# ReadAlongs/SoundSwallower

Hardware: AMD Instinct MI355X
Metric: senone-frames/sec (en-us PTM) (higher is better)
Workload: dtype f32+i32

## Files before the change

### include/ssw_amd.h

```cpp
#ifndef SSW_AMD_H
#define SSW_AMD_H

#include <stddef.h>
#include <stdint.h>

#ifdef __cplusplus
extern "C" {
#endif

#define SSW_ABI_VERSION 2

typedef struct ssw_config_s {
    double logbase;
    double varfloor;
    double mixwfloor;
    double tmatfloor;
    int32_t topn;
    int32_t ds;
    int32_t aw;
    int32_t device;
} ssw_config_t;
#define SSW_DEVICE_NONE (-2)

void ssw_config_defaults(ssw_config_t *cfg);
// ... 3 lines not shown
typedef struct ssw_model_s ssw_model_t;

ssw_model_t *ssw_model_load(const char *mdef, const char *means, const char *variances,
                            const char *sendump, const char *mixw, const char *tmat,
                            const ssw_config_t *cfg);
void ssw_model_free(ssw_model_t *m);

typedef struct ssw_model_info_s {
    int32_t n_cb, n_feat, n_density, veclen_total;
    int32_t n_sen, n_ci_sen, n_ciphone, n_phone, n_emit_state, n_tmat, n_sseq, sil;
    int32_t n_floored, topn, has_ptm, has_ms, device;
    int32_t veclen[8];
    int32_t scan_mode, mfma_selftest;
    float mfma_selftest_worst_u;
    float mfma_selftest_ms;
} ssw_model_info_t;
int ssw_model_info(const ssw_model_t *m, ssw_model_info_t *out);
const char *ssw_model_selftest_message(const ssw_model_t *m);

enum ssw_table {
    SSW_TAB_MEAN = 0, SSW_TAB_VAR, SSW_TAB_DET, SSW_TAB_PTM_MIXW, SSW_TAB_MS_PDF, SSW_TAB_TP,
    SSW_TAB_SSEQ, SSW_TAB_SEN2CB, SSW_TAB_LOGADD8, SSW_TAB_PHONE_SSID, SSW_TAB_PHONE_TMAT,
    SSW_TAB_REC, SSW_TAB_SCAN_REC, SSW_TAB_SCAN_D0, SSW_TAB_SCAN_EXACT,
    SSW_TAB_SCAN_REC_MFMA, SSW_TAB_SCAN_EXACT_MFMA, SSW_TAB_SCAN_WFRAG
};
const void *ssw_model_table(const ssw_model_t *m, int which, size_t *nbytes);

enum ssw_scorer { SSW_SCORER_PTM = 0, SSW_SCORER_MS = 1 };

int ssw_score_batch(ssw_model_t *m, int scorer, const float *d_feats, int32_t n_frames,
                    const int32_t *utt_off, int32_t n_utts, int16_t *d_out, void *stream);
#define SSW_SCORE_CARRY_UTTS 1u
#define SSW_SCORE_SHARE_DEVICE 2u
#define SSW_SCORE_CARRY_OUT_REWIND 4u
int ssw_score_batch_ex(ssw_model_t *m, int scorer, const float *d_feats, int32_t n_frames,
                       const int32_t *utt_off, int32_t n_utts, int16_t *d_out, void *stream,
                       uint32_t flags, const uint32_t *carry_in, uint32_t *carry_out);
int ssw_score_batch_host(ssw_model_t *m, int scorer, const float *feats, int32_t n_frames,
                         const int32_t *utt_off, int32_t n_utts, int16_t *out);
int ssw_score_batch_topn(ssw_model_t *m, int32_t n_frames, uint8_t *cw, int32_t *score);
int ssw_debug_mfma_f16_tiles(ssw_model_t *m, const uint16_t *A, const uint16_t *B, const float *C,
                             float *D, int32_t n_tiles);
int ssw_debug_scan_keys(ssw_model_t *m, const float *d_feats, int32_t n_frames, int32_t cbf,
                        float *keys);
int ssw_score_batch_stats(ssw_model_t *m, int64_t stats[2]);
int ssw_scan_audit_stats(ssw_model_t *m, int64_t stats[2]);

// ... 265 lines not shown
```

### soundswallower_amd/api.py

```python
from __future__ import annotations

import ctypes as C
import os

import numpy as np

from . import _lib
from ._lib import SswAlignEntry, SswConfig, SswFeConfig, SswModelInfo

SCORER_PTM = 0
SCORER_MS = 1
SSW_DEVICE_NONE = -2
INT_MAX = 2**31 - 1

_TABLES = {
    "mean": (0, np.float32), "var": (1, np.float32), "det": (2, np.float32),
    "ptm_mixw": (3, np.uint8), "ms_pdf": (4, np.uint8), "tp": (5, np.uint8),
    "sseq": (6, np.uint16), "sen2cb": (7, np.int16), "logadd8": (8, np.uint8),
    "phone_ssid": (9, np.int32), "phone_tmat": (10, np.int32),
    "rec": (11, np.float32), "scan_rec": (12, np.float32), "scan_d0": (13, np.float32),
    "scan_exact": (14, np.uint32), "scan_rec_mfma": (15, np.float32),
    "scan_exact_mfma": (16, np.uint32), "scan_wfrag": (17, np.uint16),
}


class SswError(RuntimeError):
    pass


FE_TRANSFORMS = {"legacy": 0, "dct": 1, "htk": 2}
FE_FRAME, FE_SHIFT, FE_NCEP = 410, 160, 13


def fe_frame_counts(n_samples) -> np.ndarray:
    n = np.asarray(n_samples, np.int64)
    return np.where(n <= 0, 0, np.where(n < FE_FRAME, 1, 2 + (n - FE_FRAME) // FE_SHIFT))


def fe_frame_counts_at(n_samples, samprate, frate=100, wlen=0.025625) -> np.ndarray:
    n = np.asarray(n_samples, np.int64)
    sr = np.broadcast_to(np.asarray(samprate, np.float32), n.shape)
    shift = (sr / np.float32(frate)).astype(np.float64) + 0.5
    size = (sr * np.float32(wlen)).astype(np.float64) + 0.5
    shift, size = shift.astype(np.int64), size.astype(np.int64)
    full = 1 + (n - size) // np.maximum(shift, 1)
# ... 938 lines not shown
```

### soundswallower_amd/csrc/ssw_host_model.inc

```

struct Knobs {
    int sen_fpb;
    int sen_r;
    int sen_groups;
    bool sen_generic;
    bool ms_senone_old;
    bool scan_fma;
    int mfma_min_frames;
    int score_piece;
    int host_pipe_cap;
    int mfma_steps;
    bool mfma_balance;
    int mfma_lds_pad;
    bool ptm_exact;
    bool frame_fused;
    int scan_audit;
    float selftest_eps_u;
    bool selftest_off;
    bool align_band, align_win;
    bool align_bt;
    char align_kernel[8];
    int align_band_tokens;
    int align_win_waves;
    bool align_timing;
// ... 95 lines not shown
struct ssw_model_s {
    ssw_host_model_t *h;
    Knobs kn;
    int scan_mode;
    int selftest_status;
    float selftest_worst_u, selftest_ms;
    char selftest_msg[200];
    int device;
    int n_cu;
    std::atomic<unsigned long long> owner;
    int owner_depth;
    int n_cbf, sen_stride;
    float *d_rec;
    float *d_rec28;
    float *d_recq;
    float *d_recmax;
    uint32_t *d_exlist;
    uint4 *d_wfrag;
    uint32_t *d_exlistm;
    int n_exact_form;
    uint8_t *d_mixw, *d_ms_pdf, *d_sen2cb, *d_logadd8, *d_logadd_mirror, *d_tp, *d_quad_cb;
    short4 *d_slot_sen;
    uint32_t *d_quad_info;
    uint16_t *d_sen_slot;
    unsigned char *d_act_ws;
    size_t act_ws_cap;
    int n_quads, slot_stride;
    uint32_t *d_topn_cw;
    int4 *d_topn_sc;
    int *d_utt_off;
    uint32_t *d_utt_start;
    uint32_t *d_carry0;
    size_t carry_cap;
    uint32_t *d_carry_rows;
    size_t carry_rows_cap;
    unsigned long long *d_nfixed;
    size_t ws_frames, ws_utts, ws_bits, ws_utts_hint, ws_bits_hint, meta_nw;
    std::vector<int32_t> *utt_cache;
    unsigned char *h_stage[2];
    size_t h_stage_cap[2];
    hipEvent_t ev_stage[2];
    int stage_next;
    hipStream_t last_score_stream;
    int have_last_score_stream;
    hipStream_t s_pipe, s_copy;
    hipEvent_t ev_piece[2], ev_down[2];
// ... 116 lines not shown
        }
        m->h_stage[k] = NULL;
        m->h_stage_cap[k] = 0;
        const size_t cap = (bytes + 65535) & ~(size_t)65535;
        if (hipHostMalloc((void **)&m->h_stage[k], cap, hipHostMallocDefault) != hipSuccess) {
            (void)hipGetLastError();
            ssw_set_error("hipHostMalloc(%zu) for the upload staging failed", cap);
            return NULL;
        }
        m->h_stage_cap[k] = cap;
    }
    *slot_out = k;
    return m->h_stage[k];
}

template <typename T>
static int
dev_alloc(T **p, size_t n)
{
    HIP_OK(hipMalloc(reinterpret_cast<void **>(p), n * sizeof(T)));
    return 0;
}

static int
upload_model(ssw_model_s *m)
{
    const ssw_host_model_t *h = m->h;
    const int ncbf = h->n_cb * h->n_feat;
    m->n_cbf = ncbf;
    {
        const size_t nrec = (size_t)ncbf * h->n_density * SSW_REC_FLOATS;
        const size_t nd0 = (size_t)ncbf * SSW_REC_FLOATS, nex = (size_t)ncbf * SSW_EXLIST_STRIDE;
        m->n_exact_form = h->n_exact_form;
        if (dev_alloc(&m->d_rec, nrec) < 0 || dev_alloc(&m->d_recq, nrec) < 0
            || dev_alloc(&m->d_recmax, nd0) < 0 || dev_alloc(&m->d_exlist, nex) < 0)
            return -1;
        HIP_OK(hipMemcpy(m->d_rec, h->rec, nrec * sizeof(float), hipMemcpyHostToDevice));
        HIP_OK(hipMemcpy(m->d_recq, h->recq, nrec * sizeof(float), hipMemcpyHostToDevice));
        HIP_OK(hipMemcpy(m->d_recmax, h->recd0, nd0 * sizeof(float), hipMemcpyHostToDevice));
        HIP_OK(hipMemcpy(m->d_exlist, h->exlist, nex * sizeof(uint32_t), hipMemcpyHostToDevice));
        if (h->wfrag != NULL) {
            const size_t nw = (size_t)ncbf * SSW_WFRAG_PER_CBF * sizeof(uint16_t);
            HIP_OK(hipMalloc((void **)&m->d_wfrag, nw));
            HIP_OK(hipMemcpy(m->d_wfrag, h->wfrag, nw, hipMemcpyHostToDevice));
            if (dev_alloc(&m->d_exlistm, nex) < 0
                || dev_alloc(&m->d_rec28, (size_t)ncbf * h->n_density * 28) < 0)
// ... 10 lines not shown
        int T = 0;
        for (int i = 0; i < 256; ++i)
            T = h->logadd8[i] > T ? h->logadd8[i] : T;
        std::vector<uint8_t> mir((size_t)3 * SSW_LOGADD_MIRROR);
        for (int part = 0; part < 2; ++part) {
            const int size = (part + 1) * SSW_LOGADD_MIRROR, mid = size / 2;
            uint8_t *out = mir.data() + (part ? SSW_LOGADD_MIRROR : 0);
            for (int e = 0; e < size; ++e) {
                const int d = e < mid ? mid - e : e - mid;
                out[e] = (uint8_t)(T - (d < 256 ? (int)h->logadd8[d] : 0));
            }
        }
        HIP_OK(hipMalloc((void **)&m->d_logadd_mirror, mir.size()));
        HIP_OK(hipMemcpy(m->d_logadd_mirror, mir.data(), mir.size(), hipMemcpyHostToDevice));
    }
    if (h->n_sen) {
        std::vector<uint8_t> s2c((size_t)h->n_sen);
        for (int i = 0; i < h->n_sen; ++i)
            s2c[i] = (uint8_t)h->sen2cb[i];
        HIP_OK(hipMalloc((void **)&m->d_sen2cb, s2c.size()));
        HIP_OK(hipMemcpy(m->d_sen2cb, s2c.data(), s2c.size(), hipMemcpyHostToDevice));
    }
    if (h->ptm_mixw || h->ms_pdf) {
        std::vector<int16_t> slot_sen;
        std::vector<uint8_t> quad_cb;
        for (int c = 0; c < h->n_cb; ++c) {
            size_t start = slot_sen.size();
            for (int i = 0; i < h->n_sen; ++i)
                if (h->sen2cb[i] == c)
                    slot_sen.push_back((int16_t)i);
            while ((slot_sen.size() - start) % 4)
                slot_sen.push_back(-1);
            for (size_t q = start / 4; q < slot_sen.size() / 4; ++q)
                quad_cb.push_back((uint8_t)c);
        }
        m->n_quads = (int)quad_cb.size();
        m->slot_stride = ((int)slot_sen.size() + 127) & ~127;
        m->sen_stride = m->slot_stride;
        const size_t rows = (size_t)h->n_feat * h->n_density;
        if (h->ptm_mixw) {
            std::vector<uint8_t> mw(rows * m->slot_stride, 0);
            for (size_t r = 0; r < rows; ++r)
                for (size_t sl = 0; sl < slot_sen.size(); ++sl) {
                    const int sen = slot_sen[sl] >= 0 ? slot_sen[sl] : slot_sen[sl & ~(size_t)3];
                    mw[r * m->slot_stride + sl] = h->ptm_mixw[r * h->n_sen + sen];
                }
            HIP_OK(hipMalloc((void **)&m->d_mixw, mw.size()));
            HIP_OK(hipMemcpy(m->d_mixw, mw.data(), mw.size(), hipMemcpyHostToDevice));
        }
        if (h->ms_pdf) {
            std::vector<uint8_t> mw(rows * m->slot_stride, 0);
            for (size_t sl = 0; sl < slot_sen.size(); ++sl) {
                const int sen = slot_sen[sl] >= 0 ? slot_sen[sl] : slot_sen[sl & ~(size_t)3];
                const uint8_t *src = h->ms_pdf + (size_t)sen * rows;
                for (size_t r = 0; r < rows; ++r)
                    mw[r * m->slot_stride + sl] = src[r];
            }
            HIP_OK(hipMalloc((void **)&m->d_ms_pdf, mw.size()));
            HIP_OK(hipMemcpy(m->d_ms_pdf, mw.data(), mw.size(), hipMemcpyHostToDevice));
        }
        {
            std::vector<uint32_t> qi(quad_cb.size());
            for (size_t q = 0; q < qi.size(); ++q) {
                const int16_t *sj = &slot_sen[4 * q];
                const bool run4 = sj[0] >= 0 && sj[1] == sj[0] + 1 && sj[2] == sj[0] + 2
                    && sj[3] == sj[0] + 3;
                qi[q] = ((uint32_t)sj[0] & 0xffffu) | ((uint32_t)run4 << 16)
                    | ((uint32_t)quad_cb[q] << 24);
            }
            HIP_OK(hipMalloc((void **)&m->d_quad_info, qi.size() * sizeof(uint32_t)));
            HIP_OK(hipMemcpy(m->d_quad_info, qi.data(), qi.size() * sizeof(uint32_t),
                             hipMemcpyHostToDevice));
        }
        HIP_OK(hipMalloc((void **)&m->d_quad_cb, quad_cb.size()));
        HIP_OK(hipMemcpy(m->d_quad_cb, quad_cb.data(), quad_cb.size(), hipMemcpyHostToDevice));
        {
            std::vector<uint16_t> sen_slot((size_t)h->n_sen, 0);
            for (size_t sl = 0; sl < slot_sen.size(); ++sl)
                if (slot_sen[sl] >= 0)
                    sen_slot[(size_t)slot_sen[sl]] = (uint16_t)sl;
            HIP_OK(hipMalloc((void **)&m->d_sen_slot, sen_slot.size() * sizeof(uint16_t) + 16));
            HIP_OK(hipMemcpy(m->d_sen_slot, sen_slot.data(), sen_slot.size() * sizeof(uint16_t),
                             hipMemcpyHostToDevice));
        }
        HIP_OK(hipMalloc((void **)&m->d_slot_sen, slot_sen.size() * sizeof(int16_t)));
        HIP_OK(hipMemcpy(m->d_slot_sen, slot_sen.data(), slot_sen.size() * sizeof(int16_t),
                         hipMemcpyHostToDevice));
    }
    if (h->tp) {
        size_t n = (size_t)h->tp_n_tmat * h->tp_n_state * (h->tp_n_state + 1);
        HIP_OK(hipMalloc((void **)&m->d_tp, n + 16));
        HIP_OK(hipMemcpy(m->d_tp, h->tp, n, hipMemcpyHostToDevice));
    }
    return 0;
// ... 64 lines not shown
    m->d_wfrag = NULL;
}

extern "C" ssw_model_t *
ssw_model_load(const char *mdef, const char *means, const char *variances, const char *sendump,
               const char *mixw, const char *tmat, const ssw_config_t *cfg)
{
    ssw_host_model_t *h = ssw_host_model_load(mdef, means, variances, sendump, mixw, tmat, cfg);
    if (h == NULL)
        return NULL;
    for (int f = 0; f < h->n_feat; ++f)
        if (h->veclen[f] > SSW_MAX_VECLEN) {
            ssw_set_error("stream %d has %d dimensions; the gfx950 kernels handle <= %d", f,
                          h->veclen[f], SSW_MAX_VECLEN);
            ssw_host_model_free(h);
            return NULL;
        }
    if (h->cfg.device == SSW_DEVICE_NONE) {
        ssw_model_s *hm = new ssw_model_s();
        memset(hm, 0, sizeof(*hm));
        hm->h = h;
        hm->device = SSW_DEVICE_NONE;
        hm->n_cbf = h->n_cb * h->n_feat;
        return hm;
    }
    int ndev = 0;
    if (hipGetDeviceCount(&ndev) != hipSuccess || ndev == 0) {
        ssw_set_error("no HIP device: the MI355X path has no CPU fallback");
        ssw_host_model_free(h);
        return NULL;
    }
    ssw_model_s *m = new ssw_model_s();
    memset(m, 0, sizeof(*m));
    m->h = h;
    if (h->cfg.device >= 0) {
        if (hipSetDevice(h->cfg.device) != hipSuccess) {
            ssw_set_error("hipSetDevice(%d) failed", h->cfg.device);
            ssw_model_free(m);
            return NULL;
        }
        m->device = h->cfg.device;
    } else
        (void)hipGetDevice(&m->device);
    m->n_cu = 256;
    (void)hipDeviceGetAttribute(&m->n_cu, hipDeviceAttributeMultiprocessorCount, m->device);
    if (m->n_cu <= 0)
        m->n_cu = 256;
    load_knobs(m->kn);
    if (upload_model(m) < 0) {
        ssw_model_free(m);
        return NULL;
    }
    m->force_exact = m->kn.ptm_exact;
    mfma_self_test(m);
    return m;
}

extern "C" void
ssw_model_free(ssw_model_t *m)
{
    if (m == NULL)
        return;
    if (m->device == SSW_DEVICE_NONE) {
        ssw_host_model_free(m->h);
        delete m;
        return;
    }
    (void)hipFree(m->d_rec);
    (void)hipFree(m->d_rec28);
    (void)hipFree(m->d_recq);
    (void)hipFree(m->d_recmax);
    (void)hipFree(m->d_exlist);
    (void)hipFree(m->d_wfrag);
    (void)hipFree(m->d_exlistm);
    (void)hipFree(m->d_align_ws);
    (void)hipFree(m->d_fp_ws);
    (void)hipFree(m->d_fpa_ws);
    (void)hipFree(m->d_text_scr);
    (void)hipFree(m->d_feat_off);
    (void)hipFree(m->d_fe_tab);
    if (m->fe_rate_tab)
        for (auto &kv : *m->fe_rate_tab)
            (void)hipFree(kv.second);
    delete m->fe_rate_tab;
    (void)hipFree(m->d_fe_ws);
    if (m->fe_ev_ready)
        for (int i = 0; i < 4; ++i)
            (void)hipEventDestroy(m->fe_ev[i]);
    (void)hipFree(m->d_sen_slot);
    (void)hipFree(m->d_act_ws);
    (void)hipFree(m->d_mixw);
    (void)hipFree(m->d_ms_pdf);
    (void)hipFree(m->d_sen2cb);
    if (m->s_up) {
        (void)hipEventDestroy(m->ev_up);
        (void)hipStreamDestroy(m->s_up);
    }
    (void)hipFree(m->d_quad_cb);
    (void)hipFree(m->d_quad_info);
    (void)hipFree(m->d_slot_sen);
    (void)hipFree(m->d_logadd8);
    (void)hipFree(m->d_logadd_mirror);
    (void)hipFree(m->d_tp);
    (void)hipFree(m->d_topn_cw);
    (void)hipFree(m->d_topn_sc);
    (void)hipFree(m->d_utt_off);
    (void)hipFree(m->d_carry0);
    (void)hipFree(m->d_carry_rows);
    (void)hipFree(m->d_nfixed);
    delete m->utt_cache;
    delete m->xcd_cuts;
    for (int k = 0; k < 2; ++k) {
        if (m->h_stage[k] != NULL) {
            (void)hipHostFree(m->h_stage[k]);
            (void)hipEventDestroy(m->ev_stage[k]);
        }
    }
    if (m->s_copy != NULL) {
        (void)hipStreamDestroy(m->s_copy);
        (void)hipStreamDestroy(m->s_pipe);
        for (int k = 0; k < 2; ++k) {
            (void)hipEventDestroy(m->ev_piece[k]);
// ... 62 lines not shown
{
    const ssw_host_model_t *h = m->h;
    size_t gau = (size_t)h->n_cb * h->n_density * h->veclen_total * sizeof(float);
    size_t n = 0;
    const void *p = NULL;
    switch (which) {
    case SSW_TAB_MEAN: p = h->mean; n = gau; break;
    case SSW_TAB_VAR: p = h->var; n = gau; break;
    case SSW_TAB_DET: p = h->det; n = (size_t)h->n_cb * h->n_feat * h->n_density * 4; break;
    case SSW_TAB_PTM_MIXW: p = h->ptm_mixw; n = (size_t)h->n_feat * h->n_density * h->n_sen; break;
    case SSW_TAB_MS_PDF: p = h->ms_pdf; n = (size_t)h->n_feat * h->n_density * h->n_sen; break;
    case SSW_TAB_TP: p = h->tp; n = (size_t)h->tp_n_tmat * h->tp_n_state * (h->tp_n_state + 1); break;
    case SSW_TAB_SSEQ: p = h->sseq; n = (size_t)h->n_sseq * h->n_emit_state * 2; break;
    case SSW_TAB_SEN2CB: p = h->sen2cb; n = (size_t)h->n_sen * 2; break;
    case SSW_TAB_LOGADD8: p = h->logadd8; n = 256; break;
    case SSW_TAB_PHONE_SSID: p = h->phone_ssid; n = (size_t)h->n_phone * 4; break;
    case SSW_TAB_PHONE_TMAT: p = h->phone_tmat; n = (size_t)h->n_phone * 4; break;
    case SSW_TAB_REC: p = h->rec; n = (size_t)h->n_cb * h->n_feat * h->n_density * SSW_REC_FLOATS * 4; break;
    case SSW_TAB_SCAN_REC: p = h->recq; n = (size_t)h->n_cb * h->n_feat * h->n_density * SSW_REC_FLOATS * 4; break;
    case SSW_TAB_SCAN_D0: p = h->recd0; n = (size_t)h->n_cb * h->n_feat * SSW_REC_FLOATS * 4; break;
    case SSW_TAB_SCAN_EXACT: p = h->exlist; n = (size_t)h->n_cb * h->n_feat * SSW_EXLIST_STRIDE * 4; break;
    case SSW_TAB_SCAN_REC_MFMA: p = h->recqm; n = p ? (size_t)h->n_cb * h->n_feat * h->n_density * SSW_REC_FLOATS * 4 : 0; break;
    case SSW_TAB_SCAN_EXACT_MFMA: p = h->exlistm; n = p ? (size_t)h->n_cb * h->n_feat * SSW_EXLIST_STRIDE * 4 : 0; break;
    case SSW_TAB_SCAN_WFRAG: p = h->wfrag; n = p ? (size_t)h->n_cb * h->n_feat * SSW_WFRAG_PER_CBF * 2 : 0; break;
    default: break;
    }
    if (p == NULL)
        n = 0;
    if (nbytes)
        *nbytes = n;
    return p;
}
```

### soundswallower_amd/csrc/ssw_host_score.inc

```
static int
ensure_score_ws(ssw_model_s *m, int n_frames, int n_utts)
{
    if ((size_t)n_frames > m->ws_frames) {
        (void)hipFree(m->d_topn_cw);
        (void)hipFree(m->d_topn_sc);
        m->d_topn_cw = NULL;
        m->d_topn_sc = NULL;
        m->ws_frames = 0;
        if ((uint64_t)n_frames * (uint64_t)m->n_cbf > 0xffffffffull) {
            ssw_set_error("batch of %d frames is too large (frames x codebooks x streams must fit 32 bits)",
                          n_frames);
            return -1;
        }
        if (dev_alloc(&m->d_topn_cw, (size_t)n_frames * m->n_cbf) < 0
            || dev_alloc(&m->d_topn_sc, (size_t)n_frames * m->n_cbf) < 0)
            return -1;
        m->ws_frames = (size_t)n_frames;
    }
    if (m->d_nfixed == NULL) {
        if (dev_alloc(&m->d_nfixed, 4) < 0)
            return -1;
        HIP_OK(hipMemset(m->d_nfixed, 0, 4 * sizeof(unsigned long long)));
    }
    const size_t need_bits = 2 * (((size_t)n_frames + 31) / 32 + 2);
// ... 82 lines not shown
    for (int i = 0; i < 256; ++i)
        tab_max = h->logadd8[i] > tab_max ? h->logadd8[i] : tab_max;
    return h->cfg.aw == 1 && !m->ms_raw && n_frames >= 4 * 512 && h->n_cb <= 64
        && 255 + 640 + 6 * tab_max < SSW_LOGADD_MIRROR && !m->kn.ms_senone_old;
}

static int
launch_senone(ssw_model_s *m, int scorer, int n_frames, const uint32_t *cw, const int4 *sc,
              int16_t *d_out, bool move_stats, hipStream_t st, bool share_device = false,
              const ssw_compact_plan_s *cp = NULL, int frame_base = 0)
{
    const ssw_host_model_t *h = m->h;
    SenoneParams S;
    memset(&S, 0, sizeof(S));
    S.topn_cw = cw;
    S.topn_sc = sc;
    S.mixw = scorer == SSW_SCORER_MS ? m->d_ms_pdf : m->d_mixw;
    S.aw = h->cfg.aw;
    S.zero = h->zero8;
    S.raw = m->ms_raw;
    S.quad_cb = m->d_quad_cb;
    S.quad_info = m->d_quad_info;
    S.slot_sen = m->d_slot_sen;
    S.logadd8 = m->d_logadd8;
    S.logadd_mirror = m->d_logadd_mirror + (scorer == SSW_SCORER_MS ? SSW_LOGADD_MIRROR : 0);
    S.nfixed = move_stats ? m->d_nfixed : NULL;
    S.nfixed_acc = m->stats_accumulate;
    S.out = d_out;
    if (cp != NULL) {
        S.utt_of_frame = cp->d_utt_of_frame;
        S.cutt_off = cp->d_frame_off;
        S.cstride = cp->d_cstride;
        S.crow_off = cp->d_crow_off;
        S.cpos = cp->d_cpos;
        S.frame_base = frame_base;
    }
    S.n_frames = n_frames;
    S.n_cb = h->n_cb;
    S.n_feat = h->n_feat;
    S.n_density = h->n_density;
    S.n_sen = h->n_sen;
    S.slot_stride = m->slot_stride;
    S.n_quads = m->n_quads;
    S.tab_max = 0;
    for (int i = 0; i < 256; ++i)
        S.tab_max = h->logadd8[i] > S.tab_max ? h->logadd8[i] : S.tab_max;
// ... 38 lines not shown
        case 1: SSW_MS_LAUNCH(1); break;
        case 2: SSW_MS_LAUNCH(2); break;
        case 3: SSW_MS_LAUNCH(3); break;
        case 4: SSW_MS_LAUNCH(4); break;
        default:
            ssw_set_error("too many senones (%d quads)", m->n_quads);
            return -1;
        }
#undef SSW_MS_LAUNCH
        HIP_OK(hipGetLastError());
        return 0;
    }
    if (threads < fpb * m->n_cbf)
        fpb = 1;
    if (threads < m->n_cbf) {
        ssw_set_error("unsupported senone/codebook shape (%d quads, %d codebook x stream)",
                      m->n_quads, m->n_cbf);
        return -1;
    }
    lds = (ms_packed ? 2 * SSW_LOGADD_MIRROR : SSW_LOGADD_MIRROR)
        + 3 * 4 * (size_t)(ms_packed ? ((h->n_cb + 7) & ~7) : SSW_MAX_FEAT) * fpb + 16 * sizeof(int)
        + 2 * 32 * (size_t)m->n_cbf * fpb
        + 20 * (size_t)((fpb * m->n_cbf + 63) & ~63)
        + 8 * (size_t)R * threads + 16;
    const int n_units = (n_frames + fpb - 1) / fpb;
    int per_cu = 32 / (threads / 64);
    per_cu = per_cu < 1 ? 1 : per_cu;
    int groups = m->n_cu * per_cu;
    if (share_device && groups < (n_units + 7) / 8)
        groups = (n_units + 7) / 8;
    if (kn.sen_groups >= 0)
        groups = kn.sen_groups > 0 ? kn.sen_groups : n_units;
    const dim3 grid(groups < n_units ? groups : n_units);
    const bool nf3 = h->n_feat == 3 && !kn.sen_generic;
    if (fpb != 1 && fpb != 2) {
        ssw_set_error("senone kernel: %d frames per group (1 or 2)", fpb);
        return -1;
    }
#define SSW_SEN_LAUNCH_C(RR, FP, NFV, MSV, CV)                                               \
    hipLaunchKernelGGL((ptm_senone_kernel<4, RR, FP, NFV, MSV, CV>), grid, dim3(threads), lds, st, S)
#define SSW_SEN_LAUNCH_NF(RR, FP, MSV, CV)                                                   \
    if (nf3)                                                                                 \
        SSW_SEN_LAUNCH_C(RR, FP, 3, MSV, CV);                                                \
    else                                                                                     \
        SSW_SEN_LAUNCH_C(RR, FP, 0, MSV, CV)
#define SSW_SEN_LAUNCH_FP(RR, MSV, CV)                                                       \
    if (fpb == 2) {                                                                          \
// ... 828 lines not shown
```

### soundswallower_amd/csrc/ssw_k1b_senone.inc

```

struct SenoneParams {
    const uint32_t *topn_cw;
    const int4 *topn_sc;
    const uint8_t *mixw;
    const uint8_t *quad_cb;
    const short4 *slot_sen;
    const uint32_t *quad_info;
    const uint8_t *logadd8;
    const uint8_t *logadd_mirror;
    unsigned long long *nfixed;
    int16_t *out;
    int n_frames, n_cb, n_feat, n_density, n_sen, slot_stride, n_quads;
    int aw, zero;
    int raw;
    int tab_max;
    const int32_t *utt_of_frame, *cutt_off, *cstride;
    const long long *crow_off;
    const uint32_t *cpos;
    int nfixed_acc;
    int frame_base;
};

constexpr int SEN_MAX_THREADS = 1024;

#define SSW_LOGADD_LDS 512
#define SSW_LOGADD_MIRROR 1024

__device__ __forceinline__ int
fast_logadd(int x, int y, const uint8_t *tab)
{
// ... 188 lines not shown
#define STL(k)                                                                               \
    if ((threadIdx.x & 63) == 0) {                                                           \
        int wv = blockIdx.x * 11 + (threadIdx.x >> 6);                                       \
        if (wv < 16384)                                                                      \
            g_timeline[wv * 6 + (k)] = __builtin_amdgcn_s_memtime();                        \
    }
#else
#define STL(k)
#endif
    STL(0)
    __builtin_amdgcn_s_setprio(3);
    const int n_feat = NF ? NF : P.n_feat;
    static_assert(TOPN == 4, "top-N block is packed 4 x 8 bit");
    extern __shared__ __align__(16) unsigned char smem[];
    const int n_cbf = P.n_cb * P.n_feat;
    uint8_t *s_tab = smem;
    const int NORM_W = MS ? ((P.n_cb + 7) & ~7) : SSW_MAX_FEAT;
    int *s_norm = reinterpret_cast<int *>(smem + MIRROR);
    int *s_red = s_norm + 3 * NORM_W * FPB;
    uint4 *s_item = reinterpret_cast<uint4 *>(s_red + 16);
    const int n_item_pad = (FPB * n_cbf + 63) & ~63;
    int4 *s_stage_sc = reinterpret_cast<int4 *>(s_item + 2 * 2 * n_cbf * FPB);
    uint32_t *s_stage_cw = reinterpret_cast<uint32_t *>(s_stage_sc + n_item_pad);
    short4 *s_sen4 = reinterpret_cast<short4 *>(s_stage_cw + n_item_pad);

    const int tid = threadIdx.x;
    const int nthr = blockDim.x;
    const uint32_t T = (uint32_t)P.tab_max;
    const int n_units = (P.n_frames + FPB - 1) / FPB;
    const int stride_u = (int)gridDim.x;
    int u = (int)blockIdx.x;
    if (u >= n_units)
        return;

    if ((uint32_t)(uintptr_t)(__attribute__((address_space(3))) unsigned char *)smem != 0u)
        __builtin_trap();

    uint32_t my_a, my_b;
    {
        int fr = 0;
#pragma unroll
        for (int k = 1; k < FPB; ++k)
            fr += tid >= k * n_cbf ? 1 : 0;
        const int i = tid - fr * n_cbf, f = i % n_feat;
        const int nidx = MS ? fr * NORM_W + i / n_feat : fr * SSW_MAX_FEAT + f;
        my_a = (uint32_t)fr | (uint32_t)nidx << 4 | (uint32_t)(f * P.n_density) << 16;
        my_b = (uint32_t)(2 * (i * FPB + fr));
    }
    int4 sc0 = make_int4(0, 0, 0, 0);
    uint32_t cw0 = 0;
    auto item_live = [&](int unit) {
        return tid < FPB * n_cbf && unit * FPB + (int)(my_a & 0xfu) < P.n_frames;
    };
    auto fetch_item = [&](int unit) {
        if (item_live(unit)) {
            sc0 = P.topn_sc[(size_t)unit * FPB * n_cbf + tid];
            cw0 = P.topn_cw[(size_t)unit * FPB * n_cbf + tid];
        }
    };
    auto fetch_item_dma = [&](int unit) {
        if (item_live(unit)) {
            const int4 *gsc = P.topn_sc + ((size_t)unit * FPB * n_cbf + tid);
            const uint32_t *gcw = P.topn_cw + ((size_t)unit * FPB * n_cbf + tid);
            const uint32_t wave0 = (uint32_t)tid & ~63u;
            const uint32_t dst_sc = (uint32_t)__builtin_amdgcn_readfirstlane(
                (int)((uint32_t)(uintptr_t)(__attribute__((address_space(3))) int4 *)s_stage_sc + wave0 * 16u));
            const uint32_t dst_cw = (uint32_t)__builtin_amdgcn_readfirstlane(
                (int)((uint32_t)(uintptr_t)(__attribute__((address_space(3))) uint32_t *)s_stage_cw + wave0 * 4u));
            unsigned keep;
            asm volatile("s_mov_b32 %0, m0\n\ts_mov_b32 m0, %3\n\ts_nop 0\n\t"
                         "global_load_lds_dwordx4 %1, off\n\ts_mov_b32 m0, %4\n\ts_nop 0\n\t"
                         "global_load_lds_dword %2, off\n\ts_mov_b32 m0, %0"
                         : "=&s"(keep) : "v"(gsc), "v"(gcw), "s"(dst_sc), "s"(dst_cw) : "memory");
        }
    };
    auto take_item_dma = [&](int unit) {
        asm volatile("s_waitcnt vmcnt(0)" ::: "memory");
        if (item_live(unit)) {
            sc0 = s_stage_sc[tid];
            cw0 = s_stage_cw[tid];
        }
    };
    auto norm_item = [&](int unit, int ns) {
        if (item_live(unit)) {
            int *w = &s_norm[ns * FPB * NORM_W + (int)((my_a >> 4) & 0xfffu)];
            if (MS) {
                atomicAdd(w, sc0.x);
                if (sc0.w <= P.zero + 4096)
                    atomicOr(&s_red[12 + ns], 1 << (int)(my_a & 0xfu));
            } else
                atomicMax(w, sc0.x >> SSW_SENSCR_SHIFT);
        }
    };
    auto stage_item = [&](int unit, int ns, int buf) {
        if (item_live(unit)) {
            const int norm = s_norm[ns * FPB * NORM_W + (int)((my_a >> 4) & 0xfffu)];
            const int v[4] = { sc0.x, sc0.y, sc0.z, sc0.w };
            uint32_t sp[4];
#pragma unroll
            for (int k = 0; k < TOPN; ++k) {
                int q;
                if (MS) {
                    q = v[0] - v[k];
// ... 8 lines not shown
            const uint32_t e0 = MS ? 0u : sp[0];
#pragma unroll
            for (int k = 0; k < TOPN; ++k)
                sp[k] -= e0;
            if (MS) {
                const int a0 = -norm - (int)(3u * T) * n_feat;
                if (a0 < 0 || a0 > 30000)
                    atomicOr(&s_red[12 + ns], 1 << (int)(my_a & 0xfu));
            }
            uint4 *dst = s_item + (2 * buf * n_cbf * FPB + (int)my_b);
            const uint32_t row0 = my_a >> 16;
            dst[0] = make_uint4(__umul24(row0 + (cw0 & 0xffu), (uint32_t)P.slot_stride),
                                __umul24(row0 + ((cw0 >> 8) & 0xffu), (uint32_t)P.slot_stride),
                                __umul24(row0 + ((cw0 >> 16) & 0xffu), (uint32_t)P.slot_stride),
                                __umul24(row0 + (cw0 >> 24), (uint32_t)P.slot_stride));
            reinterpret_cast<uint2 *>(dst + 1)[0]
                = make_uint2(sp[0] | (sp[1] << 16), sp[2] | (sp[3] << 16));
            reinterpret_cast<uint32_t *>(dst + 1)[2] = MS
                ? (uint32_t)((-norm - (int)(3u * T) * n_feat) & 0xffff) * 0x10001u
                : e0 * 0x10001u;
        }
    };

    fetch_item(u);
    uint32_t qi_ld[R];
    short4 sen4_ld[R];
#pragma unroll
    for (int r = 0; r < R; ++r) {
        const int q = r * nthr + tid;
        qi_ld[r] = q < P.n_quads ? P.quad_info[q] : 0u;
        sen4_ld[r] = q < P.n_quads ? P.slot_sen[q] : make_short4(-1, -1, -1, -1);
    }
    constexpr int TAB_DW = MIRROR / 4;
    uint32_t tv[(TAB_DW + 255) / 256] = {};
#pragma unroll
    for (int j = 0; j < (TAB_DW + 255) / 256; ++j) {
        const int e = tid + j * nthr;
        if (e < TAB_DW)
            tv[j] = reinterpret_cast<const uint32_t *>(P.logadd_mirror)[e];
    }
    if (tid < 3 * NORM_W * FPB)
        s_norm[tid] = MS ? 0 : SSW_WORST_SCORE;
    if (3 * NORM_W * FPB > nthr)
        for (int i = tid + nthr; i < 3 * NORM_W * FPB; i += nthr)
            s_norm[i] = MS ? 0 : SSW_WORST_SCORE;
    if (tid < 16)
        s_red[tid] = tid < 12 ? INT_MAX : 0;
    if (P.nfixed != nullptr && blockIdx.x == 0 && tid == 0) {
        P.nfixed[1] = (P.nfixed_acc ? P.nfixed[1] : 0ull) + P.nfixed[0];
        P.nfixed[0] = 0ull;
    }
    lds_barrier();
    norm_item(u, 0);
#pragma unroll
    for (int j = 0; j < (TAB_DW + 255) / 256; ++j)
        if (tid + j * nthr < TAB_DW)
            reinterpret_cast<uint32_t *>(s_tab)[tid + j * nthr] = tv[j];
    lds_barrier();
    stage_item(u, 0, 0);

    const __amdgpu_buffer_rsrc_t mw_rsrc = __builtin_amdgcn_make_buffer_rsrc(
        const_cast<uint8_t *>(P.mixw)
            + (uint32_t)__builtin_amdgcn_readfirstlane((int)((uint32_t)tid & ~63u) * 4),
        (short)4, 64, (int)(1u << 23));
    uint32_t qoff[R];
#pragma unroll
    for (int r = 0; r < R; ++r) {
        const int q = r * nthr + tid;
        const uint32_t qi = qi_ld[r];
        qoff[r] = (qi >> 24) * (uint32_t)(n_feat * FPB * 32) | ((qi >> 16) & 1u);
        s_sen4[q] = sen4_ld[r];
    }

    for (int it = 0;; ++it) {
        const int t0 = u * FPB;
        const int nfr = (P.n_frames - t0) < FPB ? (P.n_frames - t0) : FPB;
        const int u_next = u + stride_u;
        const bool has_next = u_next < n_units;
        const int buf = it & 1, slot = it % 3, slot_next = (it + 1) % 3;
        lds_barrier();
        if (has_next)
            fetch_item_dma(u_next);
        STL(1)
        uint32_t asc2[R][FPB][2];
        const uint4 *item_b = s_item + 2 * buf * n_cbf * FPB;
#pragma unroll
        for (int r = 0; r < R; ++r) {
            const int q = r * nthr + tid;
            const int soff = __builtin_amdgcn_readfirstlane(r * nthr * 4);
#pragma unroll
            for (int fr = 0; fr < FPB; ++fr) {
                const uint32_t dead = (q < P.n_quads && fr < nfr) ? 0u : 0xffffffffu;
                asc2[r][fr][0] = asc2[r][fr][1] = dead;
            }
            if (q < P.n_quads) {
                const uint4 *item_cb = reinterpret_cast<const uint4 *>(
                    reinterpret_cast<const unsigned char *>(item_b) + (qoff[r] & ~1u));
                if (MS) {
#pragma unroll
                    for (int fr = 0; fr < FPB; ++fr)
                        if (fr < nfr)
                            asc2[r][fr][0] = asc2[r][fr][1]
                                = reinterpret_cast<const uint32_t *>(item_cb + 2 * fr + 1)[2];
                }
#pragma unroll
                for (int fr = 0; fr < FPB; ++fr) {
                    {
                        constexpr int NI = R * FPB;
                        const int item = r * FPB + fr;
                        if (item * 4 < NI)
                            __builtin_amdgcn_s_setprio(3);
                        else if (item * 4 < 2 * NI)
                            __builtin_amdgcn_s_setprio(2);
                        else if (item * 4 < 3 * NI)
                            __builtin_amdgcn_s_setprio(1);
                        else
                            __builtin_amdgcn_s_setprio(0);
                    }
                    if (fr < nfr) {
                        if (NF) {
// ... 19 lines not shown
                            quad_chains<NF ? NF : 1, TOPN, MID>(mw, np, asc2[r][fr]);
                        } else
                        for (int f = 0; f < n_feat; ++f) {
                            const uint4 ro = item_cb[2 * (f * FPB + fr)];
                            const uint4 sc4 = item_cb[2 * (f * FPB + fr) + 1];
                            const uint2 np = make_uint2(sc4.x, sc4.y);
                            if (!MS) {
                                asc2[r][fr][0] += sc4.z;
                                asc2[r][fr][1] += sc4.z;
                            }
                            uint32_t mw[1][TOPN];
                            mw[0][0] = (uint32_t)__builtin_amdgcn_raw_buffer_load_b32(mw_rsrc, (int)ro.x, soff, 0);
                            mw[0][1] = (uint32_t)__builtin_amdgcn_raw_buffer_load_b32(mw_rsrc, (int)ro.y, soff, 0);
                            mw[0][2] = (uint32_t)__builtin_amdgcn_raw_buffer_load_b32(mw_rsrc, (int)ro.z, soff, 0);
                            mw[0][3] = (uint32_t)__builtin_amdgcn_raw_buffer_load_b32(mw_rsrc, (int)ro.w, soff, 0);
                            quad_chains<1, TOPN, MID>(mw, &np, asc2[r][fr]);
                        }
                    }
                }
            }
        }
        STL(2)
        __builtin_amdgcn_s_setprio(3);
        if (has_next)
            take_item_dma(u_next);
        short4 sen4[R];
#pragma unroll
        for (int r = 0; r < R; ++r)
            sen4[r] = s_sen4[r * nthr + tid];
        int c_utt[FPB];
        uint4 c_pos[R][FPB];
        if (COMPACT) {
#pragma unroll
            for (int fr = 0; fr < FPB; ++fr) {
                c_utt[fr] = fr < nfr
                    ? __builtin_amdgcn_readfirstlane(P.utt_of_frame[P.frame_base + t0 + fr]) : 0;
#pragma unroll
                for (int r = 0; r < R; ++r) {
                    const int q = r * nthr + tid;
                    c_pos[r][fr] = (q < P.n_quads && fr < nfr)
                        ? *reinterpret_cast<const uint4 *>(P.cpos + (size_t)c_utt[fr] * P.slot_stride + 4 * q)
                        : make_uint4(0xffffffffu, 0xffffffffu, 0xffffffffu, 0xffffffffu);
                }
            }
        }
#pragma unroll
        for (int fr = 0; fr < FPB; ++fr) {
            uint32_t b2 = 0xffffffffu;
#pragma unroll
            for (int r = 0; r < R; ++r)
                b2 = pk_min_u16(b2, pk_min_u16(asc2[r][fr][0], asc2[r][fr][1]));
            const int lo = (int)(b2 & 0xffffu), hi = (int)(b2 >> 16);
// ... 25 lines not shown
                    const uint32_t rb_lo = (uint32_t)__builtin_amdgcn_readfirstlane((int)(uint32_t)rb);
                    const uint32_t rb_hi = (uint32_t)__builtin_amdgcn_readfirstlane((int)(uint32_t)(rb >> 32));
                    const __amdgpu_buffer_rsrc_t orsrc = __builtin_amdgcn_make_buffer_rsrc(
                        reinterpret_cast<void *>(((uintptr_t)rb_hi << 32) | rb_lo), (short)0,
                        stride * 2, 0x00020000);
                    const uint32_t b2 = (uint32_t)best[fr] * 0x10001u;
#pragma unroll
                    for (int r = 0; r < R; ++r) {
                        const uint32_t lo2 = asc2[r][fr][0] - b2, hi2 = asc2[r][fr][1] - b2;
                        const uint4 cp = c_pos[r][fr];
                        if (cp.x != 0xffffffffu)
                            __builtin_amdgcn_raw_buffer_store_b16((short)(lo2 & 0xffffu), orsrc, (int)cp.x, 0, 0);
                        if (cp.y != 0xffffffffu)
                            asm volatile("buffer_store_short_d16_hi %0, %1, %2, 0 offen"
                                         :: "v"(lo2), "v"(cp.y), "s"(orsrc) : "memory");
                        if (cp.z != 0xffffffffu)
                            __builtin_amdgcn_raw_buffer_store_b16((short)(hi2 & 0xffffu), orsrc, (int)cp.z, 0, 0);
                        if (cp.w != 0xffffffffu)
                            asm volatile("buffer_store_short_d16_hi %0, %1, %2, 0 offen"
                                         :: "v"(hi2), "v"(cp.w), "s"(orsrc) : "memory");
                    }
                }
            }
        } else
#pragma unroll
        for (int r = 0; r < R; ++r) {
            const int q = r * nthr + tid;
            if (q < P.n_quads) {
                const bool run4 = qoff[r] & 1u;
                const int sj[4] = { sen4[r].x, sen4[r].y, sen4[r].z, sen4[r].w };
#pragma unroll
                for (int fr = 0; fr < FPB; ++fr) {
                    if (fr < nfr) {
                        const uint32_t b2 = (uint32_t)best[fr] * 0x10001u;
                        int16_t *orow = P.out + (size_t)(t0 + fr) * P.n_sen;
                        uint2u pk;
                        pk.x = asc2[r][fr][0] - b2;
                        pk.y = asc2[r][fr][1] - b2;
                        if (run4) {
                            *reinterpret_cast<uint2u *>(orow + sj[0]) = pk;
                        } else {
                            const int16_t v[4] = { (int16_t)(pk.x & 0xffffu), (int16_t)(pk.x >> 16),
                                                   (int16_t)(pk.y & 0xffffu), (int16_t)(pk.y >> 16) };
#pragma unroll
                            for (int j = 0; j < 4; ++j)
                                if (sj[j] >= 0)
                                    orow[sj[j]] = v[j];
                        }
                    }
                }
            }
        }
        STL(4)
        if (MS && marked != 0) {
            for (int fr = 0; fr < nfr; ++fr)
                if ((marked >> fr) & 1)
                    ms_exact_frame<R, COMPACT>(P, t0 + fr, tid, nthr, reinterpret_cast<int *>(s_stage_cw));
        }
        if (!has_next)
            break;
        stage_item(u_next, slot_next, buf ^ 1);
        if (tid < NORM_W * FPB)
            s_norm[slot * NORM_W * FPB + tid] = MS ? 0 : SSW_WORST_SCORE;
        if (tid < FPB)
            s_red[slot_next * FPB + tid] = INT_MAX;
        u = u_next;
    }
#undef STL
}

struct SenoneFrameParams {
    const uint32_t *topn_cw;
    const int4 *topn_sc;
    const uint8_t *mixw, *quad_cb, *logadd8;
    unsigned long long cb_mask[4];
    const uint32_t *sen_bits;
    const short4 *slot_sen;
    int16_t *out;
    int16_t *raw;
    int n_cb, n_feat, n_density, n_sen, slot_stride, n_quads;
};

struct FrameFusedParams {
// ... 466 lines not shown
```

Measured before the change: 63.77 million.

## Route non-contiguous senone quads through LDS side buffer drained by one wave

Quads whose four senones are contiguous now write their packed scores with a single global dwordx2 store at a precomputed byte offset. Quads that are not contiguous instead stage their scores into an LDS side buffer. One designated wave scatters that buffer to the output rows during the next iteration, overlapping with compute. This removes per-lane divergent 2-byte scattered stores from the main store path, at the cost of extra LDS, new model tables, and a serial drain loop on one wave.

```diff
diff --git a/include/ssw_amd.h b/include/ssw_amd.h
--- a/include/ssw_amd.h
+++ b/include/ssw_amd.h
@@ -49,7 +49,8 @@
     SSW_TAB_MEAN = 0, SSW_TAB_VAR, SSW_TAB_DET, SSW_TAB_PTM_MIXW, SSW_TAB_MS_PDF, SSW_TAB_TP,
     SSW_TAB_SSEQ, SSW_TAB_SEN2CB, SSW_TAB_LOGADD8, SSW_TAB_PHONE_SSID, SSW_TAB_PHONE_TMAT,
     SSW_TAB_REC, SSW_TAB_SCAN_REC, SSW_TAB_SCAN_D0, SSW_TAB_SCAN_EXACT,
-    SSW_TAB_SCAN_REC_MFMA, SSW_TAB_SCAN_EXACT_MFMA, SSW_TAB_SCAN_WFRAG
+    SSW_TAB_SCAN_REC_MFMA, SSW_TAB_SCAN_EXACT_MFMA, SSW_TAB_SCAN_WFRAG,
+    SSW_TAB_SLOT_SEN, SSW_TAB_SEN_SIDE
 };
 const void *ssw_model_table(const ssw_model_t *m, int which, size_t *nbytes);
 
diff --git a/soundswallower_amd/api.py b/soundswallower_amd/api.py
--- a/soundswallower_amd/api.py
+++ b/soundswallower_amd/api.py
@@ -21,6 +21,7 @@
     "rec": (11, np.float32), "scan_rec": (12, np.float32), "scan_d0": (13, np.float32),
     "scan_exact": (14, np.uint32), "scan_rec_mfma": (15, np.float32),
     "scan_exact_mfma": (16, np.uint32), "scan_wfrag": (17, np.uint16),
+    "slot_sen": (18, np.int16), "sen_side": (19, np.uint32),
 }
 
 
diff --git a/soundswallower_amd/csrc/ssw_host_model.inc b/soundswallower_amd/csrc/ssw_host_model.inc
--- a/soundswallower_amd/csrc/ssw_host_model.inc
+++ b/soundswallower_amd/csrc/ssw_host_model.inc
@@ -141,6 +141,11 @@
     uint8_t *d_mixw, *d_ms_pdf, *d_sen2cb, *d_logadd8, *d_logadd_mirror, *d_tp, *d_quad_cb;
     short4 *d_slot_sen;
     uint32_t *d_quad_info;
+    std::vector<int16_t> *slot_sen_h;
+    std::vector<uint32_t> *sen_side_h;
+    uint32_t *d_quad_out;
+    int16_t *d_side_sen;
+    int n_side;
     uint16_t *d_sen_slot;
     unsigned char *d_act_ws;
     size_t act_ws_cap;
@@ -303,6 +308,41 @@
     return 0;
 }
 
+static void
+build_slot_tables(ssw_model_s *m, std::vector<uint8_t> *quad_cb_out)
+{
+    const ssw_host_model_t *h = m->h;
+    std::vector<int16_t> &slot_sen = *(m->slot_sen_h = new std::vector<int16_t>());
+    std::vector<uint32_t> &side = *(m->sen_side_h = new std::vector<uint32_t>());
+    std::vector<uint8_t> quad_cb;
+    for (int c = 0; c < h->n_cb; ++c) {
+        size_t start = slot_sen.size();
+        for (int i = 0; i < h->n_sen; ++i)
+            if (h->sen2cb[i] == c)
+                slot_sen.push_back((int16_t)i);
+        while ((slot_sen.size() - start) % 4)
+            slot_sen.push_back(-1);
+        for (size_t q = start / 4; q < slot_sen.size() / 4; ++q)
+            quad_cb.push_back((uint8_t)c);
+    }
+    m->n_quads = (int)quad_cb.size();
+    m->n_side = 0;
+    for (size_t q = 0; q < quad_cb.size(); ++q) {
+        const int16_t *sj = &slot_sen[4 * q];
+        if (sj[0] >= 0 && sj[1] == sj[0] + 1 && sj[2] == sj[0] + 2 && sj[3] == sj[0] + 3)
+            continue;
+        ++m->n_side;
+        for (uint32_t j = 0; j < 4; ++j)
+            if (sj[j] >= 0) {
+                side.push_back((uint32_t)q);
+                side.push_back(j);
+                side.push_back((uint32_t)sj[j]);
+            }
+    }
+    if (quad_cb_out)
+        quad_cb_out->swap(quad_cb);
+}
+
 static int
 upload_model(ssw_model_s *m)
 {
@@ -359,19 +399,9 @@
         HIP_OK(hipMemcpy(m->d_sen2cb, s2c.data(), s2c.size(), hipMemcpyHostToDevice));
     }
     if (h->ptm_mixw || h->ms_pdf) {
-        std::vector<int16_t> slot_sen;
         std::vector<uint8_t> quad_cb;
-        for (int c = 0; c < h->n_cb; ++c) {
-            size_t start = slot_sen.size();
-            for (int i = 0; i < h->n_sen; ++i)
-                if (h->sen2cb[i] == c)
-                    slot_sen.push_back((int16_t)i);
-            while ((slot_sen.size() - start) % 4)
-                slot_sen.push_back(-1);
-            for (size_t q = start / 4; q < slot_sen.size() / 4; ++q)
-                quad_cb.push_back((uint8_t)c);
-        }
-        m->n_quads = (int)quad_cb.size();
+        build_slot_tables(m, &quad_cb);
+        const std::vector<int16_t> &slot_sen = *m->slot_sen_h;
         m->slot_stride = ((int)slot_sen.size() + 127) & ~127;
         m->sen_stride = m->slot_stride;
         const size_t rows = (size_t)h->n_feat * h->n_density;
@@ -407,6 +437,28 @@
             }
             HIP_OK(hipMalloc((void **)&m->d_quad_info, qi.size() * sizeof(uint32_t)));
             HIP_OK(hipMemcpy(m->d_quad_info, qi.data(), qi.size() * sizeof(uint32_t),
+                             hipMemcpyHostToDevice));
+        }
+        {
+            std::vector<uint32_t> qo(quad_cb.size());
+            std::vector<int16_t> ss(4 * (size_t)m->n_side + 2, (int16_t)-1);
+            for (size_t q = 0; q < qo.size(); ++q)
+                qo[q] = 2u * (uint32_t)slot_sen[4 * q];
+            int n = -1;
+            uint32_t last_q = 0xffffffffu;
+            for (size_t i = 0; i + 2 < m->sen_side_h->size(); i += 3) {
+                const uint32_t q = (*m->sen_side_h)[i], j = (*m->sen_side_h)[i + 1];
+                if (q != last_q) {
+                    qo[q] = 0x80000000u | (uint32_t)++n;
+                    last_q = q;
+                }
+                ss[4 * (size_t)n + j] = (int16_t)(*m->sen_side_h)[i + 2];
+            }
+            HIP_OK(hipMalloc((void **)&m->d_quad_out, qo.size() * sizeof(uint32_t)));
+            HIP_OK(hipMemcpy(m->d_quad_out, qo.data(), qo.size() * sizeof(uint32_t),
+                             hipMemcpyHostToDevice));
+            HIP_OK(hipMalloc((void **)&m->d_side_sen, ss.size() * sizeof(int16_t)));
+            HIP_OK(hipMemcpy(m->d_side_sen, ss.data(), ss.size() * sizeof(int16_t),
                              hipMemcpyHostToDevice));
         }
         HIP_OK(hipMalloc((void **)&m->d_quad_cb, quad_cb.size()));
@@ -517,6 +569,8 @@
         hm->h = h;
         hm->device = SSW_DEVICE_NONE;
         hm->n_cbf = h->n_cb * h->n_feat;
+        if (h->ptm_mixw || h->ms_pdf)
+            build_slot_tables(hm, NULL);
         return hm;
     }
     int ndev = 0;
@@ -558,6 +612,8 @@
         return;
     if (m->device == SSW_DEVICE_NONE) {
         ssw_host_model_free(m->h);
+        delete m->slot_sen_h;
+        delete m->sen_side_h;
         delete m;
         return;
     }
@@ -593,6 +649,10 @@
     }
     (void)hipFree(m->d_quad_cb);
     (void)hipFree(m->d_quad_info);
+    (void)hipFree(m->d_quad_out);
+    (void)hipFree(m->d_side_sen);
+    delete m->slot_sen_h;
+    delete m->sen_side_h;
     (void)hipFree(m->d_slot_sen);
     (void)hipFree(m->d_logadd8);
     (void)hipFree(m->d_logadd_mirror);
@@ -701,6 +761,12 @@
     case SSW_TAB_SCAN_EXACT: p = h->exlist; n = (size_t)h->n_cb * h->n_feat * SSW_EXLIST_STRIDE * 4; break;
     case SSW_TAB_SCAN_REC_MFMA: p = h->recqm; n = p ? (size_t)h->n_cb * h->n_feat * h->n_density * SSW_REC_FLOATS * 4 : 0; break;
     case SSW_TAB_SCAN_EXACT_MFMA: p = h->exlistm; n = p ? (size_t)h->n_cb * h->n_feat * SSW_EXLIST_STRIDE * 4 : 0; break;
+    case SSW_TAB_SLOT_SEN:
+        if (m->slot_sen_h) { p = m->slot_sen_h->data(); n = m->slot_sen_h->size() * 2; }
+        break;
+    case SSW_TAB_SEN_SIDE:
+        if (m->sen_side_h) { p = m->sen_side_h->data(); n = m->sen_side_h->size() * 4; }
+        break;
     case SSW_TAB_SCAN_WFRAG: p = h->wfrag; n = p ? (size_t)h->n_cb * h->n_feat * SSW_WFRAG_PER_CBF * 2 : 0; break;
     default: break;
     }
diff --git a/soundswallower_amd/csrc/ssw_host_score.inc b/soundswallower_amd/csrc/ssw_host_score.inc
--- a/soundswallower_amd/csrc/ssw_host_score.inc
+++ b/soundswallower_amd/csrc/ssw_host_score.inc
@@ -128,6 +128,9 @@
     S.quad_cb = m->d_quad_cb;
     S.quad_info = m->d_quad_info;
     S.slot_sen = m->d_slot_sen;
+    S.quad_out = m->d_quad_out;
+    S.side_sen = reinterpret_cast<const uint32_t *>(m->d_side_sen);
+    S.n_side = m->n_side;
     S.logadd8 = m->d_logadd8;
     S.logadd_mirror = m->d_logadd_mirror + (scorer == SSW_SCORER_MS ? SSW_LOGADD_MIRROR : 0);
     S.nfixed = move_stats ? m->d_nfixed : NULL;
@@ -212,7 +215,9 @@
         + 3 * 4 * (size_t)(ms_packed ? ((h->n_cb + 7) & ~7) : SSW_MAX_FEAT) * fpb + 16 * sizeof(int)
         + 2 * 32 * (size_t)m->n_cbf * fpb
         + 20 * (size_t)((fpb * m->n_cbf + 63) & ~63)
-        + 8 * (size_t)R * threads + 16;
+        + 4 * (size_t)R * threads
+        + 8 * (size_t)fpb * (m->n_side + 1)
+        + 8 * (size_t)m->n_side + 16;
     const int n_units = (n_frames + fpb - 1) / fpb;
     int per_cu = 32 / (threads / 64);
     per_cu = per_cu < 1 ? 1 : per_cu;
diff --git a/soundswallower_amd/csrc/ssw_k1b_senone.inc b/soundswallower_amd/csrc/ssw_k1b_senone.inc
--- a/soundswallower_amd/csrc/ssw_k1b_senone.inc
+++ b/soundswallower_amd/csrc/ssw_k1b_senone.inc
@@ -6,6 +6,9 @@
     const uint8_t *quad_cb;
     const short4 *slot_sen;
     const uint32_t *quad_info;
+    const uint32_t *quad_out;
+    const uint32_t *side_sen;
+    int n_side;
     const uint8_t *logadd8;
     const uint8_t *logadd_mirror;
     unsigned long long *nfixed;
@@ -240,7 +243,9 @@
     const int n_item_pad = (FPB * n_cbf + 63) & ~63;
     int4 *s_stage_sc = reinterpret_cast<int4 *>(s_item + 2 * 2 * n_cbf * FPB);
     uint32_t *s_stage_cw = reinterpret_cast<uint32_t *>(s_stage_sc + n_item_pad);
-    short4 *s_sen4 = reinterpret_cast<short4 *>(s_stage_cw + n_item_pad);
+    uint32_t *s_qout = s_stage_cw + n_item_pad;
+    unsigned char *s_side = reinterpret_cast<unsigned char *>(s_qout + R * (int)blockDim.x);
+    uint32_t *s_side_sen = reinterpret_cast<uint32_t *>(s_side + 8 * FPB * (P.n_side + 1));
 
     const int tid = threadIdx.x;
     const int nthr = blockDim.x;
@@ -267,6 +272,7 @@
     }
     int4 sc0 = make_int4(0, 0, 0, 0);
     uint32_t cw0 = 0;
+    int tq = tid;
     auto item_live = [&](int unit) {
         return tid < FPB * n_cbf && unit * FPB + (int)(my_a & 0xfu) < P.n_frames;
     };
@@ -278,9 +284,9 @@
     };
     auto fetch_item_dma = [&](int unit) {
         if (item_live(unit)) {
-            const int4 *gsc = P.topn_sc + ((size_t)unit * FPB * n_cbf + tid);
-            const uint32_t *gcw = P.topn_cw + ((size_t)unit * FPB * n_cbf + tid);
-            const uint32_t wave0 = (uint32_t)tid & ~63u;
+            const int4 *gsc = P.topn_sc + ((size_t)unit * FPB * n_cbf + tq);
+            const uint32_t *gcw = P.topn_cw + ((size_t)unit * FPB * n_cbf + tq);
+            const uint32_t wave0 = (uint32_t)tq & ~63u;
             const uint32_t dst_sc = (uint32_t)__builtin_amdgcn_readfirstlane(
                 (int)((uint32_t)(uintptr_t)(__attribute__((address_space(3))) int4 *)s_stage_sc + wave0 * 16u));
             const uint32_t dst_cw = (uint32_t)__builtin_amdgcn_readfirstlane(
@@ -295,8 +301,8 @@
     auto take_item_dma = [&](int unit) {
         asm volatile("s_waitcnt vmcnt(0)" ::: "memory");
         if (item_live(unit)) {
-            sc0 = s_stage_sc[tid];
-            cw0 = s_stage_cw[tid];
+            sc0 = s_stage_sc[tq];
+            cw0 = s_stage_cw[tq];
         }
     };
     auto norm_item = [&](int unit, int ns) {
@@ -351,14 +357,19 @@
         }
     };
 
+    uint32_t qo_ld[R];
+#pragma unroll
+    for (int r = 0; r < R; ++r) {
+        const int q = r * nthr + tid;
+        qo_ld[r] = !COMPACT && q < P.n_quads ? P.quad_out[q] : 0x80000000u | (uint32_t)P.n_side;
+    }
+    const uint32_t ss_ld = !COMPACT && tid < 2 * P.n_side ? P.side_sen[tid] : 0u;
     fetch_item(u);
     uint32_t qi_ld[R];
-    short4 sen4_ld[R];
 #pragma unroll
     for (int r = 0; r < R; ++r) {
         const int q = r * nthr + tid;
         qi_ld[r] = q < P.n_quads ? P.quad_info[q] : 0u;
-        sen4_ld[r] = q < P.n_quads ? P.slot_sen[q] : make_short4(-1, -1, -1, -1);
     }
     constexpr int TAB_DW = MIRROR / 4;
     uint32_t tv[(TAB_DW + 255) / 256] = {};
@@ -381,6 +392,14 @@
     }
     lds_barrier();
     norm_item(u, 0);
+    if (!COMPACT) {
+#pragma unroll
+        for (int r = 0; r < R; ++r)
+            s_qout[r * nthr + tid] = (int)qo_ld[r] < 0
+                ? 0x80000000u + (qo_ld[r] & 0x7fffffffu) * (8u * FPB) : qo_ld[r];
+        if (tid < 2 * P.n_side)
+            s_side_sen[tid] = ss_ld;
+    }
 #pragma unroll
     for (int j = 0; j < (TAB_DW + 255) / 256; ++j)
         if (tid + j * nthr < TAB_DW)
@@ -395,11 +414,34 @@
     uint32_t qoff[R];
 #pragma unroll
     for (int r = 0; r < R; ++r) {
-        const int q = r * nthr + tid;
         const uint32_t qi = qi_ld[r];
-        qoff[r] = (qi >> 24) * (uint32_t)(n_feat * FPB * 32) | ((qi >> 16) & 1u);
-        s_sen4[q] = sen4_ld[r];
-    }
+        qoff[r] = (qi >> 24) * (uint32_t)(n_feat * FPB * 32);
+    }
+    if (!COMPACT) {
+        if (2 * P.n_side > nthr)
+            for (int i = tid + nthr; i < 2 * P.n_side; i += nthr)
+                s_side_sen[i] = P.side_sen[i];
+    }
+    auto drain_side = [&](int t0d, int nfrd, int skip) {
+        int lane = tid & 63;
+        asm volatile("" : "+v"(lane));
+#pragma unroll 1
+        for (int fr = 0; fr < nfrd; ++fr) {
+            if ((skip >> fr) & 1)
+                continue;
+            char *orow = reinterpret_cast<char *>(P.out + (size_t)(t0d + fr) * P.n_sen);
+#pragma unroll 1
+            for (int i = lane; i < 4 * P.n_side; i += 64) {
+                const int sen = reinterpret_cast<const int16_t *>(s_side_sen)[i];
+                const uint16_t v = *reinterpret_cast<const uint16_t *>(
+                    s_side + (i >> 2) * (8 * FPB) + fr * 8 + (i & 3) * 2);
+                if (sen >= 0)
+                    *reinterpret_cast<uint16_t *>(orow + (uint32_t)sen * 2u) = v;
+            }
+        }
+    };
+    const bool drain_wave = __builtin_amdgcn_readfirstlane(tid >> 6) == (nthr >> 6) - 1;
+    int prev_marked = 0;
 
     for (int it = 0;; ++it) {
         const int t0 = u * FPB;
@@ -408,8 +450,11 @@
         const bool has_next = u_next < n_units;
         const int buf = it & 1, slot = it % 3, slot_next = (it + 1) % 3;
         lds_barrier();
+        asm volatile("" : "+v"(tq), "+v"(my_a), "+v"(my_b));
         if (has_next)
             fetch_item_dma(u_next);
+        if (!COMPACT && it > 0 && drain_wave)
+            drain_side(t0 - stride_u * FPB, FPB, prev_marked);
         STL(1)
         uint32_t asc2[R][FPB][2];
         const uint4 *item_b = s_item + 2 * buf * n_cbf * FPB;
@@ -424,7 +469,7 @@
             }
             if (q < P.n_quads) {
                 const uint4 *item_cb = reinterpret_cast<const uint4 *>(
-                    reinterpret_cast<const unsigned char *>(item_b) + (qoff[r] & ~1u));
+                    reinterpret_cast<const unsigned char *>(item_b) + qoff[r]);
                 if (MS) {
 #pragma unroll
                     for (int fr = 0; fr < FPB; ++fr)
@@ -490,12 +535,15 @@
         }
         STL(2)
         __builtin_amdgcn_s_setprio(3);
+        asm volatile("" : "+v"(tq), "+v"(my_a), "+v"(my_b));
         if (has_next)
             take_item_dma(u_next);
-        short4 sen4[R];
-#pragma unroll
-        for (int r = 0; r < R; ++r)
-            sen4[r] = s_sen4[r * nthr + tid];
+        uint32_t qout[R];
+        if (!COMPACT) {
+#pragma unroll
+            for (int r = 0; r < R; ++r)
+                qout[r] = s_qout[r * nthr + tid];
+        }
         int c_utt[FPB];
         uint4 c_pos[R][FPB];
         if (COMPACT) {
@@ -567,32 +615,41 @@
                     }
                 }
             }
-        } else
-#pragma unroll
-        for (int r = 0; r < R; ++r) {
-            const int q = r * nthr + tid;
-            if (q < P.n_quads) {
-                const bool run4 = qoff[r] & 1u;
-                const int sj[4] = { sen4[r].x, sen4[r].y, sen4[r].z, sen4[r].w };
+        } else {
+            uint32_t b2[FPB];
+            char *orow[FPB];
+            const uint32_t side_bias
+                = (uint32_t)(uintptr_t)(__attribute__((address_space(3))) unsigned char *)s_side
+                - 0x80000000u;
+#pragma unroll
+            for (int fr = 0; fr < FPB; ++fr) {
+                b2[fr] = (uint32_t)best[fr] * 0x10001u;
+                orow[fr] = reinterpret_cast<char *>(P.out + (size_t)(t0 + fr) * P.n_sen);
+            }
+#pragma unroll
+            for (int r = 0; r < R; ++r) {
+                uint2u pk[FPB];
 #pragma unroll
                 for (int fr = 0; fr < FPB; ++fr) {
-                    if (fr < nfr) {
-                        const uint32_t b2 = (uint32_t)best[fr] * 0x10001u;
-                        int16_t *orow = P.out + (size_t)(t0 + fr) * P.n_sen;
-                        uint2u pk;
-                        pk.x = asc2[r][fr][0] - b2;
-                        pk.y = asc2[r][fr][1] - b2;
-                        if (run4) {
-                            *reinterpret_cast<uint2u *>(orow + sj[0]) = pk;
-                        } else {
-                            const int16_t v[4] = { (int16_t)(pk.x & 0xffffu), (int16_t)(pk.x >> 16),
-                                                   (int16_t)(pk.y & 0xffffu), (int16_t)(pk.y >> 16) };
-#pragma unroll
-                            for (int j = 0; j < 4; ++j)
-                                if (sj[j] >= 0)
-                                    orow[sj[j]] = v[j];
-                        }
-                    }
+                    pk[fr].x = asc2[r][fr][0] - b2[fr];
+                    pk[fr].y = asc2[r][fr][1] - b2[fr];
+                }
+                if ((int)qout[r] >= 0) {
+#pragma unroll
+                    for (int fr = 0; fr < FPB; ++fr)
+                        if (fr < nfr)
+                            asm volatile("global_store_dwordx2 %0, %1, %2"
+                                         :: "v"(qout[r]), "v"(pk[fr]), "s"(orow[fr]) : "memory");
+                } else {
+                    unsigned char *e = (unsigned char *)(
+                        __attribute__((address_space(3))) unsigned char *)(uintptr_t)(
+                        side_bias + qout[r]);
+                    if constexpr (FPB == 2)
+                        *reinterpret_cast<uint4 *>(e) = make_uint4(pk[0].x, pk[0].y, pk[1].x, pk[1].y);
+                    else
+#pragma unroll
+                        for (int fr = 0; fr < FPB; ++fr)
+                            *reinterpret_cast<uint2 *>(e + 8 * fr) = make_uint2(pk[fr].x, pk[fr].y);
                 }
             }
         }
@@ -602,8 +659,15 @@
                 if ((marked >> fr) & 1)
                     ms_exact_frame<R, COMPACT>(P, t0 + fr, tid, nthr, reinterpret_cast<int *>(s_stage_cw));
         }
-        if (!has_next)
+        if (!has_next) {
+            if (!COMPACT) {
+                lds_barrier();
+                if (drain_wave)
+                    drain_side(t0, nfr, marked);
+            }
             break;
+        }
+        prev_marked = marked;
         stage_item(u_next, slot_next, buf ^ 1);
         if (tid < NORM_W * FPB)
             s_norm[slot * NORM_W * FPB + tid] = MS ? 0 : SSW_WORST_SCORE;
```

New measurement: 63.17 million (median of 2 runs). About the same (-1.0%).
